# caishiqing/voice-tts

Measured on AMD Instinct MI355X. Metric: audio_seconds_per_second, higher is better.
Workload: dtype bf16

## Files before the change

voice-tts_amd/csrc/gemm_x6.hip:

```cpp
#include "common.h"

namespace ixtts {

typedef float gx_f32x16 __attribute__((ext_vector_type(16)));
typedef __bf16 gx_bf16x8 __attribute__((ext_vector_type(8)));
typedef float gx_f32x4 __attribute__((ext_vector_type(4)));
typedef unsigned int gx_u32x4 __attribute__((ext_vector_type(4)));


__global__ void gemm_x6_pack_kernel(const float* __restrict__ w, uint4* __restrict__ out, int N, int K, int Npad) {
  const long total = (long)(K / 8) * Npad;
  for (long idx = blockIdx.x * (long)blockDim.x + threadIdx.x; idx < total; idx += (long)gridDim.x * blockDim.x) {
    const int n = (int)(idx % Npad);
    const int ko = (int)(idx / Npad);
    float v[8];
#pragma unroll
    for (int e = 0; e < 8; ++e) v[e] = n < N ? w[(long)n * K + ko * 8 + e] : 0.f;
    uint4 ph, pm, pl;
    split8_bf16x3(v, ph, pm, pl);
    const int g = ko >> 1, kh = ko & 1;
    uint4* base = out + ((long)g * 6) * Npad + n;
    base[(long)(0 * 2 + kh) * Npad] = ph;
    base[(long)(1 * 2 + kh) * Npad] = pm;
    base[(long)(2 * 2 + kh) * Npad] = pl;
  }
}

__global__ __launch_bounds__(256) void gemm_x6_split_kernel(const float* __restrict__ a, long lda, uint4* __restrict__ out, int M, int K, long Mpad) {
  __shared__ float tile[64][65];
  const int r0 = blockIdx.x * 64, k0 = blockIdx.y * 64;
  const int t = threadIdx.x;
#pragma unroll
  for (int i = 0; i < 4; ++i) {
    const int r = (t >> 4) + 16 * i, kq = t & 15;
    float4 v = make_float4(0.f, 0.f, 0.f, 0.f);
    if (r0 + r < M) v = *reinterpret_cast<const float4*>(a + (long)(r0 + r) * lda + k0 + 4 * kq);
    tile[r][4 * kq + 0] = v.x; tile[r][4 * kq + 1] = v.y; tile[r][4 * kq + 2] = v.z; tile[r][4 * kq + 3] = v.w;
  }
  __syncthreads();
#pragma unroll
  for (int u = 0; u < 2; ++u) {
    const int r = t & 63, o = (t >> 6) + 4 * u;
    float v[8];
#pragma unroll
    for (int e = 0; e < 8; ++e) v[e] = tile[r][o * 8 + e];
    uint4 ph, pm, pl;
    split8_bf16x3(v, ph, pm, pl);
    const int ko = (k0 >> 3) + o, g = ko >> 1, kh = ko & 1;
    uint4* base = out + ((long)g * 6) * Mpad + r0 + r;
    base[(long)(0 * 2 + kh) * Mpad] = ph;
    base[(long)(1 * 2 + kh) * Mpad] = pm;
    base[(long)(2 * 2 + kh) * Mpad] = pl;
  }
}

struct GemmX6Params {
  const uint4* Ap;
  long Mpad;
  long arow0;
  const uint4* Wp;
  const float* bias;
  float* C;
  long ldc;
  int M, N, Npad, K, accumulate, m_tiles, n_tiles;
  unsigned long long* dbg;
};


template <int MT, int NT, int NST, int DBG = 0>
__global__ __launch_bounds__(256, (NST * (MT + NT) * 6 * 64 * 16 <= 80 * 1024) ? 2 : 1) void gemm_x6_kernel(GemmX6Params p) {
  constexpr int BM = 64 * MT, BN = 64 * NT;
  constexpr int A_UNITS = 6 * BM, W_UNITS = 6 * BN, STAGE = A_UNITS + W_UNITS;
  constexpr int NDMA = (6 * (MT + NT)) / 4;
  static_assert((6 * (MT + NT)) % 4 == 0, "the copies are dealt evenly to the 4 waves");
  constexpr int D = NST - 1;
  extern __shared__ uint4 smem[];

  const int nwg = p.m_tiles * p.n_tiles;
  const int bid = blockIdx.x;
  const int xcd = bid & 7, idx = bid >> 3;
  const int qd = nwg >> 3, rm = nwg & 7;
  const int lin = (xcd < rm ? xcd * (qd + 1) : rm * (qd + 1) + (xcd - rm) * qd) + idx;
  const int m_tile = lin / p.n_tiles, n_tile = lin - m_tile * p.n_tiles;
  const int m0 = m_tile * BM, n0 = n_tile * BN;

  const int tid = threadIdx.x, lane = tid & 63, wave = tid >> 6;
  const int wm = wave >> 1, wn = wave & 1;
  const int l31 = lane & 31, lh = lane >> 5;

  gx_f32x16 acc[MT][NT];
#pragma unroll
  for (int i = 0; i < MT; ++i)
#pragma unroll
    for (int j = 0; j < NT; ++j)
#pragma unroll
      for (int r = 0; r < 16; ++r) acc[i][j][r] = 0.f;

  const uint4* asrc = p.Ap + p.arow0 + m0 + lane;
  const uint4* wsrc = p.Wp + n0 + lane;
  auto issue = [&](int s, uint4* st) {
#pragma unroll
    for (int q = 0; q < NDMA; ++q) {
      const int e = q * 4 + wave;
      if (e < 6 * MT) {
        const int run = e / MT, piece = e % MT;
        __builtin_amdgcn_global_load_lds((const __attribute__((address_space(1))) void*)(asrc + ((long)s * 6 + run) * p.Mpad + piece * 64),
                                         (__attribute__((address_space(3))) void*)(st + run * BM + piece * 64), 16, 0, 0);
      } else {
        const int e2 = e - 6 * MT, run = e2 / NT, piece = e2 % NT;
        __builtin_amdgcn_global_load_lds((const __attribute__((address_space(1))) void*)(wsrc + ((long)s * 6 + run) * p.Npad + piece * 64),
                                         (__attribute__((address_space(3))) void*)(st + A_UNITS + run * BN + piece * 64), 16, 0, 0);
      }
    }
  };

  const int steps = p.K >> 4;
  auto wg_stamp = [&](int k) {
    if constexpr (DBG == 3) {
      if (tid == 0) p.dbg[128 + (long)blockIdx.x * 4 + k] = __builtin_amdgcn_s_memrealtime();
    }
  };
  auto wait_younger = [&](int y) {
    if (y >= 2) asm volatile("s_waitcnt vmcnt(%0)" ::"n"(2 * NDMA) : "memory");
    else if (y == 1) asm volatile("s_waitcnt vmcnt(%0)" ::"n"(NDMA) : "memory");
    else asm volatile("s_waitcnt vmcnt(0)" ::: "memory");
  };
  static_assert(D >= 1 && D <= 3, "1..3 steps of copies in flight behind the one waited for");
  wg_stamp(0);
  for (int t = 0; t < D && t < steps; ++t) issue(t, smem + t * STAGE);
  wait_younger(min(D, steps) - 1);
  __builtin_amdgcn_s_barrier();
  asm volatile("" ::: "memory");
  wg_stamp(1);

  const unsigned base_addr = (unsigned)(uintptr_t)(const __attribute__((address_space(3))) void*)smem;
  int st_cur = 0, st_nxt = D % NST;
  for (int s = 0; s < steps; ++s) {
    auto stamp = [&](int k) {
      if constexpr (DBG == 3) {
        if (blockIdx.x == 0 && tid == 0 && s < 16) {
          p.dbg[s * 8 + k] = __builtin_amdgcn_s_memtime();
          if (k == 0) p.dbg[s * 8 + 7] = __builtin_amdgcn_s_memrealtime();
        }
      }
    };
    stamp(0);
    if (DBG != 1 && s + D < steps) issue(s + D, smem + st_nxt * STAGE);
    stamp(1);
    const unsigned cur_addr = base_addr + (unsigned)(st_cur * STAGE * 16);
    if constexpr (DBG != 2) {
      gx_u32x4 af[3][MT], bf[3][NT];
      const unsigned aaddr = cur_addr + (unsigned)((lh * BM + wm * (32 * MT) + l31) * 16);
      const unsigned waddr = cur_addr + (unsigned)((A_UNITS + lh * BN + wn * (32 * NT) + l31) * 16);
      if constexpr (MT == 4 && NT == 2) {
        asm volatile(
            "ds_read_b128 %0, %18 offset:%20\n ds_read_b128 %1, %18 offset:%21\n ds_read_b128 %2, %18 offset:%22\n ds_read_b128 %3, %18 offset:%23\n"
            "ds_read_b128 %4, %18 offset:%24\n ds_read_b128 %5, %18 offset:%25\n ds_read_b128 %6, %18 offset:%26\n ds_read_b128 %7, %18 offset:%27\n"
            "ds_read_b128 %8, %18 offset:%28\n ds_read_b128 %9, %18 offset:%29\n ds_read_b128 %10, %18 offset:%30\n ds_read_b128 %11, %18 offset:%31\n"
            "ds_read_b128 %12, %19 offset:%32\n ds_read_b128 %13, %19 offset:%33\n ds_read_b128 %14, %19 offset:%34\n ds_read_b128 %15, %19 offset:%35\n"
            "ds_read_b128 %16, %19 offset:%36\n ds_read_b128 %17, %19 offset:%37\n s_waitcnt lgkmcnt(0)"
            : "=&v"(af[0][0]), "=&v"(af[0][1]), "=&v"(af[0][2]), "=&v"(af[0][3]), "=&v"(af[1][0]), "=&v"(af[1][1]), "=&v"(af[1][2]), "=&v"(af[1][3]),
              "=&v"(af[2][0]), "=&v"(af[2][1]), "=&v"(af[2][2]), "=&v"(af[2][3]), "=&v"(bf[0][0]), "=&v"(bf[0][1]), "=&v"(bf[1][0]), "=&v"(bf[1][1]),
              "=&v"(bf[2][0]), "=&v"(bf[2][1])
            : "v"(aaddr), "v"(waddr), "n"((0 * 2 * BM + 0) * 16), "n"((0 * 2 * BM + 32) * 16), "n"((0 * 2 * BM + 64) * 16), "n"((0 * 2 * BM + 96) * 16),
              "n"((1 * 2 * BM + 0) * 16), "n"((1 * 2 * BM + 32) * 16), "n"((1 * 2 * BM + 64) * 16), "n"((1 * 2 * BM + 96) * 16), "n"((2 * 2 * BM + 0) * 16),
              "n"((2 * 2 * BM + 32) * 16), "n"((2 * 2 * BM + 64) * 16), "n"((2 * 2 * BM + 96) * 16), "n"((0 * 2 * BN + 0) * 16), "n"((0 * 2 * BN + 32) * 16),
              "n"((1 * 2 * BN + 0) * 16), "n"((1 * 2 * BN + 32) * 16), "n"((2 * 2 * BN + 0) * 16), "n"((2 * 2 * BN + 32) * 16)
            : "memory");
      } else {
        static_assert(MT == 2 && NT == 2, "fragment block written for 256 x 128 and 128 x 128 tiles");
        asm volatile(
            "ds_read_b128 %0, %12 offset:%14\n ds_read_b128 %1, %12 offset:%15\n ds_read_b128 %2, %12 offset:%16\n ds_read_b128 %3, %12 offset:%17\n"
            "ds_read_b128 %4, %12 offset:%18\n ds_read_b128 %5, %12 offset:%19\n ds_read_b128 %6, %13 offset:%20\n ds_read_b128 %7, %13 offset:%21\n"
            "ds_read_b128 %8, %13 offset:%22\n ds_read_b128 %9, %13 offset:%23\n ds_read_b128 %10, %13 offset:%24\n ds_read_b128 %11, %13 offset:%25\n"
            "s_waitcnt lgkmcnt(0)"
            : "=&v"(af[0][0]), "=&v"(af[0][1]), "=&v"(af[1][0]), "=&v"(af[1][1]), "=&v"(af[2][0]), "=&v"(af[2][1]), "=&v"(bf[0][0]), "=&v"(bf[0][1]),
              "=&v"(bf[1][0]), "=&v"(bf[1][1]), "=&v"(bf[2][0]), "=&v"(bf[2][1])
            : "v"(aaddr), "v"(waddr), "n"((0 * 2 * BM + 0) * 16), "n"((0 * 2 * BM + 32) * 16), "n"((1 * 2 * BM + 0) * 16), "n"((1 * 2 * BM + 32) * 16),
              "n"((2 * 2 * BM + 0) * 16), "n"((2 * 2 * BM + 32) * 16), "n"((0 * 2 * BN + 0) * 16), "n"((0 * 2 * BN + 32) * 16), "n"((1 * 2 * BN + 0) * 16),
              "n"((1 * 2 * BN + 32) * 16), "n"((2 * 2 * BN + 0) * 16), "n"((2 * 2 * BN + 32) * 16)
            : "memory");
      }
      stamp(2);
#pragma unroll
      for (int i = 0; i < MT; ++i)
#pragma unroll
        for (int j = 0; j < NT; ++j) {
          const gx_bf16x8 ah = __builtin_bit_cast(gx_bf16x8, af[0][i]), am = __builtin_bit_cast(gx_bf16x8, af[1][i]), al = __builtin_bit_cast(gx_bf16x8, af[2][i]);
          const gx_bf16x8 bh = __builtin_bit_cast(gx_bf16x8, bf[0][j]), bm = __builtin_bit_cast(gx_bf16x8, bf[1][j]), bl = __builtin_bit_cast(gx_bf16x8, bf[2][j]);
          acc[i][j] = __builtin_amdgcn_mfma_f32_32x32x16_bf16(al, bh, acc[i][j], 0, 0, 0);
          acc[i][j] = __builtin_amdgcn_mfma_f32_32x32x16_bf16(ah, bl, acc[i][j], 0, 0, 0);
          acc[i][j] = __builtin_amdgcn_mfma_f32_32x32x16_bf16(am, bm, acc[i][j], 0, 0, 0);
          acc[i][j] = __builtin_amdgcn_mfma_f32_32x32x16_bf16(am, bh, acc[i][j], 0, 0, 0);
          acc[i][j] = __builtin_amdgcn_mfma_f32_32x32x16_bf16(ah, bm, acc[i][j], 0, 0, 0);
          acc[i][j] = __builtin_amdgcn_mfma_f32_32x32x16_bf16(ah, bh, acc[i][j], 0, 0, 0);
        }
      if constexpr (DBG == 3) asm volatile("" ::"v"(acc[0][0][0]), "v"(acc[MT - 1][NT - 1][15]));
    }
    stamp(3);
    wait_younger(DBG == 1 ? 0 : max(0, min(D - 1, steps - s - 2)));
    stamp(4);
    __builtin_amdgcn_s_barrier();
    asm volatile("" ::: "memory");
    stamp(5);
    st_cur = st_cur + 1 == NST ? 0 : st_cur + 1;
    st_nxt = st_nxt + 1 == NST ? 0 : st_nxt + 1;
  }

  wg_stamp(2);
#pragma unroll
  for (int j = 0; j < NT; ++j) {
    const int col = n0 + wn * (32 * NT) + j * 32 + l31;
    const bool col_ok = col < p.N;
    const float bv = (p.bias != nullptr && col_ok) ? p.bias[col] : 0.f;
#pragma unroll
    for (int i = 0; i < MT; ++i) {
      const int rbase = m0 + wm * (32 * MT) + i * 32 + 4 * lh;
#pragma unroll
      for (int r = 0; r < 16; ++r) {
        const int row = rbase + (r & 3) + 8 * (r >> 2);
        if (col_ok && row < p.M) {
          float* c = p.C + (long)row * p.ldc + col;
          float v = acc[i][j][r] + bv;
          if (p.accumulate) v += *c;
          *c = v;
        }
      }
    }
  }
  if constexpr (DBG == 3) {
    asm volatile("s_waitcnt vmcnt(0)" ::: "memory");
    wg_stamp(3);
  }
}

template <int MT, int NT, int NST, int DBG = 0>
static int launch_gemm_x6(GemmX6Params p, hipStream_t st) {
  constexpr int BM = 64 * MT, BN = 64 * NT;
  constexpr size_t smem = (size_t)NST * (6 * BM + 6 * BN) * 16;
  static_assert(smem <= 160 * 1024, "LDS stages of this tile shape");
  p.m_tiles = ceil_div(p.M, BM);
  p.n_tiles = ceil_div(p.N, BN);
  IX_ARG((long)p.n_tiles * BN <= p.Npad, "gemm_x6: packed weights padded to %d features, the %d-wide tile needs %d", p.Npad, BN, p.n_tiles * BN);
  IX_ARG(p.arow0 + (long)p.m_tiles * BM <= p.Mpad, "gemm_x6: activation planes hold %ld rows, the %d-row tiles reach row %ld", p.Mpad, BM, p.arow0 + (long)p.m_tiles * BM);
  auto kern = gemm_x6_kernel<MT, NT, NST, DBG>;
  static bool done = false;
  if (!done) {
    IX_HIP(hipFuncSetAttribute((const void*)kern, hipFuncAttributeMaxDynamicSharedMemorySize, (int)smem));
    done = true;
  }
  hipLaunchKernelGGL(kern, dim3(p.m_tiles * p.n_tiles), dim3(256), smem, st, p);
  IX_HIP(hipGetLastError());
  return IXTTS_OK;
}

}

using namespace ixtts;

extern "C" size_t ixtts_gemm_x6_packed_bytes(int N, int K) {
  if (N <= 0 || K <= 0 || K % 64) return 0;
  const size_t Npad = (size_t)(N + 255) / 256 * 256;
  return (size_t)(K / 16) * 6 * Npad * 16;
}

extern "C" int ixtts_gemm_x6_pack(const float* w_dev, void* packed_dev, int N, int K, void* stream) {
  IX_ARG(w_dev && packed_dev && N > 0 && K > 0 && K % 64 == 0, "gemm_x6_pack: bad argument (K must be a multiple of 64)");
  const int Npad = (N + 255) / 256 * 256;
  const long total = (long)(K / 8) * Npad;
  hipLaunchKernelGGL(gemm_x6_pack_kernel, dim3((unsigned)std::min<long>((total + 255) / 256, 4096)), dim3(256), 0, (hipStream_t)stream, w_dev,
                     reinterpret_cast<uint4*>(packed_dev), N, K, Npad);
  IX_HIP(hipGetLastError());
  return IXTTS_OK;
}

extern "C" long ixtts_gemm_x6_rows_padded(long rows) { return rows <= 0 ? 0 : (rows + 255) / 256 * 256 + 256; }

extern "C" int ixtts_gemm_x6_split(const float* a_dev, long lda, void* planes_dev, long rows, int K, void* stream) {
  IX_ARG(a_dev && planes_dev && rows > 0 && K > 0 && K % 64 == 0, "gemm_x6_split: bad argument (K must be a multiple of 64)");
  IX_ARG(lda >= K && lda % 4 == 0 && (reinterpret_cast<uintptr_t>(a_dev) & 15) == 0, "gemm_x6_split: rows must be 16-byte aligned (lda %ld)", lda);
  const long Mpad = ixtts_gemm_x6_rows_padded(rows);
  hipLaunchKernelGGL(gemm_x6_split_kernel, dim3((unsigned)(Mpad / 64), K / 64), dim3(256), 0, (hipStream_t)stream, a_dev, lda,
                     reinterpret_cast<uint4*>(planes_dev), (int)rows, K, Mpad);
  IX_HIP(hipGetLastError());
  return IXTTS_OK;
}

extern "C" int ixtts_gemm_x6_f32(const void* a_planes_dev, long rows_total, long row0, const void* packed_dev, const float* bias_dev, float* c_dev,
                                 long ldc, int M, int N, int K, int accumulate, int tile, void* stream) {
  IX_ARG(a_planes_dev && packed_dev && c_dev && M > 0 && N > 0 && K > 0 && K % 64 == 0, "gemm_x6: bad argument (K must be a multiple of 64: the split pass works on 64-wide k blocks)");
  IX_ARG(ldc >= N && row0 >= 0 && row0 + M <= rows_total, "gemm_x6: rows [%ld, %ld) of %ld, ldc %ld", row0, row0 + M, rows_total, ldc);
  GemmX6Params p;
  p.Ap = reinterpret_cast<const uint4*>(a_planes_dev); p.Mpad = ixtts_gemm_x6_rows_padded(rows_total); p.arow0 = row0;
  p.Wp = reinterpret_cast<const uint4*>(packed_dev); p.bias = bias_dev; p.C = c_dev; p.ldc = ldc;
  p.M = M; p.N = N; p.Npad = (N + 255) / 256 * 256; p.K = K; p.accumulate = accumulate ? 1 : 0; p.m_tiles = p.n_tiles = 0;
  p.dbg = (tile == 32 || tile == 33) ? reinterpret_cast<unsigned long long*>(const_cast<float*>(bias_dev)) : nullptr;
  if (p.dbg) p.bias = nullptr;
  hipStream_t st = (hipStream_t)stream;
  if (tile == 0) {
    const long t42 = (long)ceil_div(M, 256) * ceil_div(N, 128);
    tile = t42 >= 140 ? 2 : 3;
  }
  switch (tile) {
    case 2: return launch_gemm_x6<4, 2, 2>(p, st);
    case 3: return launch_gemm_x6<2, 2, 3>(p, st);
    case 4: return launch_gemm_x6<4, 2, 4>(p, st);
    case 5: return launch_gemm_x6<2, 2, 4>(p, st);
    case 12: return launch_gemm_x6<4, 2, 2, 1>(p, st);
    case 22: return launch_gemm_x6<4, 2, 2, 2>(p, st);
    case 32: return launch_gemm_x6<4, 2, 2, 3>(p, st);
    case 33: return launch_gemm_x6<2, 2, 3, 3>(p, st);
  }
  set_error("gemm_x6: tile %d (0 auto; 2 / 3: 256x128 / 128x128, two workgroups per CU; 4 / 5: the same, one per CU with a 4-stage ring)", tile);
  return IXTTS_ERR_ARG;
}
```

voice-tts_amd/s2mel.py:

```python
import math
import os

import torch
import torch.nn.functional as F

from .convs import conv1d

from .weights import fold_weight_norm

S2MEL_CFG = dict(
    hidden_dim=512, num_heads=8, depth=13, in_channels=80, content_dim=512, style_dim=192,
    wavenet_hidden=512, wavenet_layers=8, wavenet_kernel=5, wavenet_dilation_rate=1,
    lr_channels=512, lr_in_channels=1024, lr_n_blocks=4, gpt_dim=1280, codebook_dim=8, codebook_size=8192, semantic_dim=1024,
)


def tiny_s2mel_cfg(**kw):
    c = dict(S2MEL_CFG)
    c.update(hidden_dim=64, num_heads=2, depth=5, content_dim=32, style_dim=12, wavenet_hidden=64, wavenet_layers=3,
             lr_channels=32, lr_in_channels=40, lr_n_blocks=2, gpt_dim=128, codebook_size=8194, semantic_dim=40)
    c.update(kw)
    return c


# ... 90 lines not shown
    ws = torch.empty(nws, device=q.device, dtype=torch.uint8)
    with torch.cuda.device(q.device):
        rc = L.ixtts_attn_full_f32(q.data_ptr(), k.data_ptr(), v.data_ptr(), out.data_ptr(), B, Hh, T, d, q.stride(0), q.stride(1),
                                   q.stride(2), out.stride(0), out.stride(1), out.stride(2), C.c_float(sc), ws.data_ptr(), nws,
                                   _lib.current_stream_ptr())
    _lib.check(rc, "ixtts_attn_full_f32")
    return out


def _lin(x, W, name):
    return F.linear(x, W[name + ".weight"], W.get(name + ".bias"))


def _hip_call(name, *args):
    from . import _lib

    _lib.check(getattr(_lib.lib(), name)(*args, _lib.current_stream_ptr()), name)


def adaln_rmsnorm(x, wb, g, eps=1e-5):
    B, T, H = x.shape
    if x.is_cuda:
        import ctypes as C

        x, wb = x.contiguous(), wb.contiguous()
        out = torch.empty_like(x)
        with torch.cuda.device(x.device):
            _hip_call("ixtts_adaln_rmsnorm_f32", x.data_ptr(), wb.data_ptr(), g.data_ptr(), out.data_ptr(), B, T, H, C.c_float(eps))
        return out
    w, b = wb[:, None, :H], wb[:, None, H:]
    return torch.addcmul(b, w, F.rms_norm(x, (H,), g, eps))


def ln_modulate(x, ss, eps=1e-6):
    B, T, H = x.shape
    if x.is_cuda:
        import ctypes as C

        x, ss = x.contiguous(), ss.contiguous()
        out = torch.empty_like(x)
        with torch.cuda.device(x.device):
            _hip_call("ixtts_ln_modulate_f32", x.data_ptr(), ss.data_ptr(), out.data_ptr(), B, T, H, C.c_float(eps))
        return out
    return F.layer_norm(x, (H,), None, None, eps) * (1 + ss[:, None, H:]) + ss[:, None, :H]


def swiglu(u):
    Fd = u.shape[-1] // 2
    if u.is_cuda:
        u = u.contiguous()
        out = torch.empty(*u.shape[:-1], Fd, device=u.device, dtype=u.dtype)
        with torch.cuda.device(u.device):
            _hip_call("ixtts_swiglu_f32", u.data_ptr(), out.data_ptr(), u.numel() // (2 * Fd), Fd)
        return out
    return F.silu(u[..., :Fd]) * u[..., Fd:]


def wn_gate(a, g, off, C_):
    B, _, T = a.shape
    if a.is_cuda:
        a, g = a.contiguous(), g.contiguous()
        out = torch.empty(B, C_, T, device=a.device, dtype=a.dtype)
        with torch.cuda.device(a.device):
            _hip_call("ixtts_wn_gate_f32", a.data_ptr(), g.data_ptr(), out.data_ptr(), B, C_, T, g.shape[1], off)
        return out
    x = a + g[:, off:off + 2 * C_, None]
    return torch.tanh(x[:, :C_]) * torch.sigmoid(x[:, C_:])


def wn_gate_rows(a, g, off, C_, rows_per_batch):
    rows, B = a.shape[0], g.shape[0]
    if a.is_cuda:
        a, g = a.contiguous(), g.contiguous()
        out = torch.empty(rows, C_, device=a.device, dtype=a.dtype)
        with torch.cuda.device(a.device):
            _hip_call("ixtts_wn_gate_rows_f32", a.data_ptr(), g.data_ptr(), out.data_ptr(), rows, C_, rows_per_batch, B, g.shape[1], off)
        return out
    b = (torch.arange(rows, device=a.device) // rows_per_batch).clamp(max=B - 1)
    x = a + g[b, off:off + 2 * C_]
    return torch.tanh(x[:, :C_]) * torch.sigmoid(x[:, C_:])


def reflect_halo_rows(p, T, left, right):
    B, _, C_ = p.shape
    if p.is_cuda:
        assert p.is_contiguous()
        with torch.cuda.device(p.device):
            _hip_call("ixtts_reflect_halo_rows_f32", p.data_ptr(), B, T, C_, left, right)
        return p
    if left:
        p[:, :left] = p[:, left + 1:2 * left + 1].flip(1)
    if right:
        p[:, left + T:] = p[:, left + T - 1 - right:left + T - 1].flip(1)
    return p


TUNED_GEMMS = os.path.join(os.path.dirname(os.path.abspath(__file__)), "tunable", "gfx950_s2mel.csv")


def use_tuned_gemms(path=TUNED_GEMMS):
    if not torch.cuda.is_available():
        return False
    import torch.cuda.tunable as tn

    tn.enable(True)
    tn.tuning_enable(os.environ.get("IXTTS_TUNE") == "1")
    try:
        import tempfile

        tn.set_filename(os.path.join(tempfile.gettempdir(), "ixtts_tunableop_online.csv"))
    except Exception:
        pass
    try:
        return bool(os.path.isfile(path) and tn.read_file(path))
    except Exception:
        return False


_TUNED_T0, _TUNED_TH0 = 2322, 1909
_tuned_lengths = set()


def extend_tuned_gemms(T, Th, path=TUNED_GEMMS):
    if (T, Th) in _tuned_lengths or (T, Th) == (_TUNED_T0, _TUNED_TH0):
        return False
    _tuned_lengths.add((T, Th))
    import tempfile

    import torch.cuda.tunable as tn

    sub = {str(2 * _TUNED_T0): str(2 * T), str(_TUNED_T0): str(T), str(_TUNED_TH0): str(Th), str(2 * _TUNED_TH0): str(2 * Th),
           str(2 * _TUNED_TH0 + 4): str(2 * Th + 4)}
    head, rows = [], []
    for line in open(path).read().splitlines():
        f = line.split(",")
        if f[0] == "Validator":
            head.append(line)
        elif len(f) >= 4 and f[2] != "Default" and f[0].endswith("_TN"):
            toks = f[1].split("_")
            if any(t in sub for t in toks):
                rows.append(",".join([f[0], "_".join(sub.get(t, t) for t in toks)] + f[2:]))
    if not rows:
        return False
    with tempfile.NamedTemporaryFile("w", suffix=".csv", delete=False) as fh:
        fh.write("\n".join(head + rows) + "\n")
    try:
        return bool(tn.read_file(fh.name))
    except Exception:
        return False
    finally:
        os.unlink(fh.name)


class S2Mel:
    def __init__(self, W, cfg=S2MEL_CFG, device="cpu"):
        self.cfg = dict(cfg)
        self.device = torch.device(device)
        self.tuned_gemms = False
        if self.device.type == "cuda" and os.environ.get("IXTTS_NO_TUNED_GEMMS") != "1":
            self.tuned_gemms = use_tuned_gemms()
        W = fold_weight_norm(dict(W))
        self.W = {k: v.to(self.device, torch.float32) for k, v in W.items()}
        H = cfg["hidden_dim"]
        self.head_dim = H // cfg["num_heads"]
        half = 128
        self.t_freqs = torch.exp(-math.log(10000.0) * torch.arange(half, dtype=torch.float32) / half).to(self.device)
        self._rope = None
        W, C_, L = self.W, cfg["in_channels"], cfg["depth"]
        t = "cfm.estimator.transformer."
        self.w13 = [torch.cat([W[t + f"layers.{i}.feed_forward.w1.weight"], W[t + f"layers.{i}.feed_forward.w3.weight"]], 0).contiguous() for i in range(L)]
        self.skip_w = {i: (W[t + f"layers.{i}.skip_in_linear.weight"][:, :H].contiguous(), W[t + f"layers.{i}.skip_in_linear.weight"][:, H:].contiguous())
                       for i in range(L // 2 + 1, L)}
        names = [t + f"layers.{i}.{n}" for i in range(L) for n in ("attention_norm", "ffn_norm")] + [t + "norm"]
        self.proj_w = torch.cat([W[n + ".project_layer.weight"] for n in names], 0).contiguous()
        self.proj_b = torch.cat([W[n + ".project_layer.bias"] for n in names], 0).contiguous()
        mw = W["cfm.estimator.cond_x_merge_linear.weight"]
        self.merge_x, self.merge_rest = mw[:, :C_].contiguous(), mw[:, C_:].contiguous()
        wn = "cfm.estimator.wavenet."
        self.wn_taps = [[W[wn + f"in_layers.{i}.conv.conv.weight"][:, :, j].contiguous() for j in range(cfg["wavenet_kernel"])]
                        for i in range(cfg["wavenet_layers"])]
        nl, Hw = cfg["wavenet_layers"], cfg["wavenet_hidden"]
        self.wn_r1, self.wn_r2, self.wn_bin = [], [], []
        carry = torch.zeros(Hw, device=self.device)
        self.wn_out_bias = torch.zeros(Hw, device=self.device)
        for i in range(nl):
            rw, rb = W[wn + f"res_skip_layers.{i}.conv.conv.weight"][:, :, 0], W[wn + f"res_skip_layers.{i}.conv.conv.bias"]
            self.wn_bin.append(W[wn + f"in_layers.{i}.conv.conv.bias"] + sum(self.wn_taps[i]) @ carry)
            if i < nl - 1:
                self.wn_r1.append(rw[:Hw].contiguous())
                self.wn_r2.append(rw[Hw:].contiguous())
                carry = carry + rb[:Hw]
                self.wn_out_bias = self.wn_out_bias + rb[Hw:]
            else:
                self.wn_r1.append(None)
                self.wn_r2.append(rw.contiguous())
                self.wn_out_bias = self.wn_out_bias + rb
        sw = W["cfm.estimator.skip_linear.weight"]
        self.skipl_res, self.skipl_x = sw[:, :H].contiguous(), sw[:, H:].contiguous()

    def gpt_layer(self, latent):
        x = _lin(latent, self.W, "gpt_layer.0")
        x = _lin(x, self.W, "gpt_layer.1")
        return _lin(x, self.W, "gpt_layer.2")

    def vq2emb(self, codes):
        emb = self.W["quantizer.codebook.weight"][codes.long()]
        out = conv1d(emb.transpose(1, 2), self.W["quantizer.out_project.weight"], self.W["quantizer.out_project.bias"])
        return out.transpose(1, 2)

    def length_regulator(self, x, ylens):
        W = self.W
        x = _lin(x, W, "length_regulator.content_in_proj")
        T = int(ylens.max())
        x = F.interpolate(x.transpose(1, 2).contiguous(), size=T, mode="nearest")
        for i in range(self.cfg["lr_n_blocks"]):
            x = conv1d(x, W[f"length_regulator.model.{3 * i}.weight"], W[f"length_regulator.model.{3 * i}.bias"], padding=1)
            x = F.group_norm(x, 1, W[f"length_regulator.model.{3 * i + 1}.weight"], W[f"length_regulator.model.{3 * i + 1}.bias"], 1e-5)
            x = F.mish(x)
        n = 3 * self.cfg["lr_n_blocks"]
        x = conv1d(x, W[f"length_regulator.model.{n}.weight"], W[f"length_regulator.model.{n}.bias"])
        mask = (torch.arange(T, device=x.device).unsqueeze(0) < ylens.unsqueeze(1)).unsqueeze(-1)
        return x.transpose(1, 2) * mask

    def _t_embed(self, t, prefix):
        args = 1000.0 * t[:, None].float() * self.t_freqs[None]
        emb = torch.cat([torch.cos(args), torch.sin(args)], dim=-1)
        h = F.silu(_lin(emb, self.W, prefix + ".mlp.0"))
        return _lin(h, self.W, prefix + ".mlp.2")

    def _rope_cache(self, T):
        if self._rope is None or self._rope.shape[0] < T:
            n = self.head_dim
            freqs = 1.0 / (10000.0 ** (torch.arange(0, n, 2)[: n // 2].float() / n))
            ang = torch.outer(torch.arange(max(T, 64)).float(), freqs)
            self._rope = torch.polar(torch.ones_like(ang), ang).to(self.device)
        return self._rope[:T]

    @staticmethod
    def _rotary(x, fc):
        xc = torch.view_as_complex(x.reshape(*x.shape[:-1], -1, 2))
        return torch.view_as_real(xc * fc.view(1, fc.shape[0], 1, fc.shape[1])).flatten(3)

    def _attention(self, qkv, B, T, mask):
        H, nh, hd = self.cfg["hidden_dim"], self.cfg["num_heads"], self.head_dim
        fc = self._rope_cache(T)
        if mask is None and hd == 64 and qkv.is_cuda:
            with torch.cuda.device(qkv.device):
                _hip_call("ixtts_rope_qk_f32", qkv.data_ptr(), torch.view_as_real(fc).data_ptr(), B, T, H, hd)
            v4 = qkv.view(B, T, 3, nh, hd)
            return attn_full(v4[:, :, 0], v4[:, :, 1], v4[:, :, 2]).reshape(B * T, H)
        q, k, v = qkv.view(B, T, 3 * H).split([H, H, H], dim=-1)
        q = self._rotary(q.reshape(B, T, nh, hd), fc)
        k = self._rotary(k.reshape(B, T, nh, hd), fc)
        v = v.reshape(B, T, nh, hd)
        y = F.scaled_dot_product_attention(q.transpose(1, 2), k.transpose(1, 2), v.transpose(1, 2), attn_mask=mask, dropout_p=0.0)
        return y.transpose(1, 2).reshape(B * T, H)

    def _transformer(self, x, c, mask):
        W, cfg = self.W, self.cfg
        B, T, H = x.shape
        L = cfg["depth"]
        wb_all = F.linear(c, self.proj_w, self.proj_b).view(B, 2 * L + 1, 2 * H).transpose(0, 1).contiguous()
        x = x.reshape(B * T, H)
        skips = []
        for i in range(L):
            p = f"cfm.estimator.transformer.layers.{i}."
            if i > L // 2:
                wa, wb_ = self.skip_w[i]
                x = F.linear(skips.pop(), wb_, W[p + "skip_in_linear.bias"]).addmm_(x, wa.t())
            a = adaln_rmsnorm(x.view(B, T, H), wb_all[2 * i], W[p + "attention_norm.norm.weight"])
            y = self._attention(F.linear(a.view(B * T, H), W[p + "attention.wqkv.weight"]), B, T, mask)
            h = torch.addmm(x, y, W[p + "attention.wo.weight"].t()) if 0 < i <= L // 2 else x.addmm_(y, W[p + "attention.wo.weight"].t())
            f = adaln_rmsnorm(h.view(B, T, H), wb_all[2 * i + 1], W[p + "ffn_norm.norm.weight"])
            x = h.addmm_(swiglu(F.linear(f.view(B * T, H), self.w13[i])), W[p + "feed_forward.w2.weight"].t())
            if i < L // 2:
                skips.append(x)
        return adaln_rmsnorm(x.view(B, T, H), wb_all[2 * L], W["cfm.estimator.transformer.norm.norm.weight"])

    def _wavenet(self, x, x_mask, g, full):
        W, cfg = self.W, self.cfg
        Hw, nl, k = cfg["wavenet_hidden"], cfg["wavenet_layers"], cfg["wavenet_kernel"]
        p = "cfm.estimator.wavenet."
        g = F.linear(g, W[p + "cond_layer.conv.conv.weight"][:, :, 0], W[p + "cond_layer.conv.conv.bias"])
        out = None
        for i in range(nl):
            d = cfg["wavenet_dilation_rate"] ** i
            tot = (k - 1) * d
            right = tot // 2
            xin = _pad_reflect(x, tot - right, right)
            if x.is_cuda:
                wk, T_ = self.wn_taps[i], x.shape[-1]
                acc = W[p + f"in_layers.{i}.conv.conv.bias"][None, :, None].expand(x.shape[0], -1, T_)
                for j in range(k):
                    wj, xj = wk[j].expand(x.shape[0], -1, -1), xin[:, :, j * d:j * d + T_]
                    acc = torch.baddbmm(acc, wj, xj) if j == 0 else acc.baddbmm_(wj, xj)
                xin = acc
            else:
                xin = conv1d(xin, W[p + f"in_layers.{i}.conv.conv.weight"], W[p + f"in_layers.{i}.conv.conv.bias"], dilation=d)
            acts = wn_gate(xin, g, i * 2 * Hw, Hw)
            rs = conv1d(acts, W[p + f"res_skip_layers.{i}.conv.conv.weight"], W[p + f"res_skip_layers.{i}.conv.conv.bias"])
            if i < nl - 1:
                x = x + rs[:, :Hw]
                if not full:
                    x = x * x_mask
                out = rs[:, Hw:] if out is None else out + rs[:, Hw:]
            else:
                out = rs if out is None else out + rs
        return out if full else out * x_mask

    def _wavenet_gemm(self, x, g):
        W, cfg = self.W, self.cfg
        Hw, nl, k = cfg["wavenet_hidden"], cfg["wavenet_layers"], cfg["wavenet_kernel"]
        B, _, T_ = x.shape
        p = "cfm.estimator.wavenet."
        g = F.linear(g, W[p + "cond_layer.conv.conv.weight"][:, :, 0], W[p + "cond_layer.conv.conv.bias"])
        x = x.contiguous()
        out = None
        for i in range(nl):
            d = cfg["wavenet_dilation_rate"] ** i
            tot = (k - 1) * d
            right = tot // 2
            xin = _pad_reflect(x, tot - right, right)
            acc = self.wn_bin[i][None, :, None].expand(B, -1, T_)
            for j in range(k):
                wj, xj = self.wn_taps[i][j].expand(B, -1, -1), xin[:, :, j * d:j * d + T_]
                acc = torch.baddbmm(acc, wj, xj) if j == 0 else acc.baddbmm_(wj, xj)
            acts = wn_gate(acc, g, i * 2 * Hw, Hw)
            if i < nl - 1:
                x = x.baddbmm_(self.wn_r1[i].expand(B, -1, -1), acts)
            r2 = self.wn_r2[i].expand(B, -1, -1)
            out = torch.bmm(r2, acts) if out is None else out.baddbmm_(r2, acts)
        return out

    def _wavenet_rows(self, h, g):
        W, cfg = self.W, self.cfg
        Hw, nl, k = cfg["wavenet_hidden"], cfg["wavenet_layers"], cfg["wavenet_kernel"]
        assert cfg["wavenet_dilation_rate"] == 1
        B, T_, _ = h.shape
        p = "cfm.estimator.wavenet."
        g = F.linear(g, W[p + "cond_layer.conv.conv.weight"][:, :, 0], W[p + "cond_layer.conv.conv.bias"])
        tot = k - 1
        right = tot // 2
        left = tot - right
        Tp = T_ + tot
        P = torch.empty(B, Tp, Hw, device=h.device, dtype=h.dtype)
        P[:, left:left + T_] = h
        P2 = P.view(B * Tp, Hw)
        M = B * Tp - tot
        centre = P2[left:left + M]
        out = torch.empty(B * Tp, Hw, device=h.device, dtype=h.dtype)
        for i in range(nl):
            reflect_halo_rows(P, T_, left, right)
            acc = torch.addmm(self.wn_bin[i], P2[:M], self.wn_taps[i][0].t())
            for j in range(1, k):
                acc.addmm_(P2[j:j + M], self.wn_taps[i][j].t())
            acts = wn_gate_rows(acc, g, i * 2 * Hw, Hw, Tp)
            if i < nl - 1:
                centre.addmm_(acts, self.wn_r1[i].t())
            if i == 0:
                torch.mm(acts, self.wn_r2[i].t(), out=out[:M])
            else:
                out[:M].addmm_(acts, self.wn_r2[i].t())
        return out.view(B, Tp, Hw)[:, :T_]

    def dit_prepare(self, prompt_x, x_lens, style, cond):
        W = self.W
        e = "cfm.estimator."
        B, _, T = prompt_x.shape
        cond = _lin(cond, W, e + "cond_projection")
        rest = torch.cat([prompt_x.transpose(1, 2), cond, style[:, None, :].expand(B, T, style.shape[-1])], dim=-1)
        base = F.linear(rest, self.merge_rest, W[e + "cond_x_merge_linear.bias"])
        x_mask = (torch.arange(T, device=prompt_x.device).unsqueeze(0) < x_lens.unsqueeze(1)).unsqueeze(1)
        full = int(x_lens.min()) >= T
        if full:
            attn_mask = None
        else:
            attn_mask = x_mask[:, None, :].expand(x_mask.shape[0], 1, T, T)
            if attn_mask.shape[0] != B:
                attn_mask = attn_mask.expand(B, 1, T, T)
        return dict(B=B, T=T, base=base, x_mask=x_mask.to(base.dtype), attn_mask=attn_mask, full=full)

    def dit_step(self, ctx, x, t, out_from=0):
        W, cfg = self.W, self.cfg
        e = "cfm.estimator."
        B, T, base = ctx["B"], ctx["T"], ctx["base"]
        xt = x.transpose(1, 2)
        t1 = self._t_embed(t, e + "t_embedder")
        x_in = base + F.linear(xt, self.merge_x)
        x_res = self._transformer(x_in, t1, ctx["attn_mask"])
        halo = sum((cfg["wavenet_kernel"] - 1) * cfg["wavenet_dilation_rate"] ** i for i in range(cfg["wavenet_layers"])) // 2 + 1
        lo = max(0, out_from - halo) if (ctx["full"] and out_from > 0) else 0
        if lo > 0:
            x_res, xt = x_res[:, lo:], xt[:, lo:]
        Th = T - lo
        if self.tuned_gemms and os.environ.get("IXTTS_TUNED_ANY_LENGTH", "1") == "1":
            extend_tuned_gemms(T, Th)
        x_res = F.linear(x_res, self.skipl_res, W[e + "skip_linear.bias"]) + F.linear(xt, self.skipl_x)
        h = _lin(x_res, W, e + "conv1")
        t2 = self._t_embed(t, e + "t_embedder2")
        gemm_form = h.is_cuda and ctx["full"] and Th > 2 * cfg["wavenet_kernel"] * cfg["wavenet_dilation_rate"] ** (cfg["wavenet_layers"] - 1)
        if gemm_form and cfg["wavenet_dilation_rate"] == 1:
            h = self._wavenet_rows(h, t2) + F.linear(x_res, W[e + "res_projection.weight"], W[e + "res_projection.bias"] + self.wn_out_bias)
        elif gemm_form:
            h = self._wavenet_gemm(h.transpose(1, 2), t2).transpose(1, 2) + F.linear(x_res, W[e + "res_projection.weight"],
                                                                                     W[e + "res_projection.bias"] + self.wn_out_bias)
        else:
            mask = ctx["x_mask"][:, :, lo:] if lo > 0 else ctx["x_mask"]
            h = self._wavenet(h.transpose(1, 2), mask, t2, ctx["full"]).transpose(1, 2) + _lin(x_res, W, e + "res_projection")
        ss = _lin(F.silu(t1), W, e + "final_layer.adaLN_modulation.1")
        h = ln_modulate(h, ss)
        h = _lin(h, W, e + "final_layer.linear").transpose(1, 2)
        out = conv1d(h, W[e + "conv2.weight"], W[e + "conv2.bias"])
        return out[:, :, out_from - lo:] if out_from > 0 else out

    def dit(self, x, prompt_x, x_lens, t, style, cond):
        return self.dit_step(self.dit_prepare(prompt_x, x_lens, style, cond), x, t)

    @torch.no_grad()
    def cfm_inference(self, mu, x_lens, prompt, style, n_timesteps=25, inference_cfg_rate=0.7, noise=None, temperature=1.0):
        B, T = mu.shape[0], mu.shape[1]
        assert B == 1, "CFM inference is batch-1 (as the reference)"
        z = (torch.randn(B, self.cfg["in_channels"], T, device=mu.device) if noise is None else noise.to(mu.device, torch.float32)) * temperature
        t_span = torch.linspace(0, 1, n_timesteps + 1, device=mu.device)
        x = z.clone()
        Tp = prompt.shape[-1]
        prompt_x = torch.zeros_like(x)
        prompt_x[..., :Tp] = prompt[..., :Tp]
# ... 34 lines not shown
```

Measured before the change: 39.78.

## Route S2Mel wqkv and w13 projections through split-bf16 x6 GEMM with 8-wave tiles

Generalizes the x6 GEMM kernel to configurable wave grids (WM x WN) and adds 8-wave 256x256 and 256x128 tile variants. S2Mel now pre-packs the wqkv and fused w1/w3 weights into the three-way bf16 split format. It sends those projections through the x6 kernel, choosing the tile by row count, instead of the fp32 library linear. The aim is to replace fp32 GEMMs with MFMA-based emulated-fp32 matmuls, at the cost of extra packing memory and activation packing per call.

Result: faster. 40.19 (median of 6 runs) (+1.0%).

```diff
diff --git a/voice-tts_amd/csrc/gemm_x6.hip b/voice-tts_amd/csrc/gemm_x6.hip
--- a/voice-tts_amd/csrc/gemm_x6.hip
+++ b/voice-tts_amd/csrc/gemm_x6.hip
@@ -67,12 +67,15 @@
 };
 
 
-template <int MT, int NT, int NST, int DBG = 0>
-__global__ __launch_bounds__(256, (NST * (MT + NT) * 6 * 64 * 16 <= 80 * 1024) ? 2 : 1) void gemm_x6_kernel(GemmX6Params p) {
-  constexpr int BM = 64 * MT, BN = 64 * NT;
+template <int MT, int NT, int NST, int DBG = 0, int WM = 2, int WN = 2>
+__global__ __launch_bounds__(64 * WM * WN, WM * WN > 4 ? 1 : (NST * (MT + NT) * 6 * 64 * 16 <= 80 * 1024) ? 2 : 1) void gemm_x6_kernel(GemmX6Params p) {
+  constexpr int NW = WM * WN;
+  constexpr int BM = 32 * MT * WM, BN = 32 * NT * WN;
   constexpr int A_UNITS = 6 * BM, W_UNITS = 6 * BN, STAGE = A_UNITS + W_UNITS;
-  constexpr int NDMA = (6 * (MT + NT)) / 4;
-  static_assert((6 * (MT + NT)) % 4 == 0, "the copies are dealt evenly to the 4 waves");
+  constexpr int PA = BM / 64, PW = BN / 64;
+  constexpr int NPIECE = 6 * (PA + PW);
+  constexpr int NDMA = (NPIECE + NW - 1) / NW;
+  static_assert(BM % 64 == 0 && BN % 64 == 0, "tiles of whole 64-unit pieces");
   constexpr int D = NST - 1;
   extern __shared__ uint4 smem[];
 
@@ -85,7 +88,7 @@
   const int m0 = m_tile * BM, n0 = n_tile * BN;
 
   const int tid = threadIdx.x, lane = tid & 63, wave = tid >> 6;
-  const int wm = wave >> 1, wn = wave & 1;
+  const int wm = wave / WN, wn = wave % WN;
   const int l31 = lane & 31, lh = lane >> 5;
 
   gx_f32x16 acc[MT][NT];
@@ -101,13 +104,13 @@
   auto issue = [&](int s, uint4* st) {
 #pragma unroll
     for (int q = 0; q < NDMA; ++q) {
-      const int e = q * 4 + wave;
-      if (e < 6 * MT) {
-        const int run = e / MT, piece = e % MT;
+      const int e = min(q * NW + wave, NPIECE - 1);
+      if (e < 6 * PA) {
+        const int run = e / PA, piece = e % PA;
         __builtin_amdgcn_global_load_lds((const __attribute__((address_space(1))) void*)(asrc + ((long)s * 6 + run) * p.Mpad + piece * 64),
                                          (__attribute__((address_space(3))) void*)(st + run * BM + piece * 64), 16, 0, 0);
       } else {
-        const int e2 = e - 6 * MT, run = e2 / NT, piece = e2 % NT;
+        const int e2 = e - 6 * PA, run = e2 / PW, piece = e2 % PW;
         __builtin_amdgcn_global_load_lds((const __attribute__((address_space(1))) void*)(wsrc + ((long)s * 6 + run) * p.Npad + piece * 64),
                                          (__attribute__((address_space(3))) void*)(st + A_UNITS + run * BN + piece * 64), 16, 0, 0);
       }
@@ -133,6 +136,54 @@
   asm volatile("" ::: "memory");
   wg_stamp(1);
 
+  auto read_frags = [&](unsigned cur_addr, gx_u32x4 (&af)[3][MT], gx_u32x4 (&bf)[3][NT]) {
+    const unsigned aaddr = cur_addr + (unsigned)((lh * BM + wm * (32 * MT) + l31) * 16);
+    const unsigned waddr = cur_addr + (unsigned)((A_UNITS + lh * BN + wn * (32 * NT) + l31) * 16);
+    if constexpr (MT == 4 && NT == 2) {
+      asm volatile(
+          "ds_read_b128 %0, %18 offset:%20\n ds_read_b128 %1, %18 offset:%21\n ds_read_b128 %2, %18 offset:%22\n ds_read_b128 %3, %18 offset:%23\n"
+          "ds_read_b128 %4, %18 offset:%24\n ds_read_b128 %5, %18 offset:%25\n ds_read_b128 %6, %18 offset:%26\n ds_read_b128 %7, %18 offset:%27\n"
+          "ds_read_b128 %8, %18 offset:%28\n ds_read_b128 %9, %18 offset:%29\n ds_read_b128 %10, %18 offset:%30\n ds_read_b128 %11, %18 offset:%31\n"
+          "ds_read_b128 %12, %19 offset:%32\n ds_read_b128 %13, %19 offset:%33\n ds_read_b128 %14, %19 offset:%34\n ds_read_b128 %15, %19 offset:%35\n"
+          "ds_read_b128 %16, %19 offset:%36\n ds_read_b128 %17, %19 offset:%37\n s_waitcnt lgkmcnt(0)"
+          : "=&v"(af[0][0]), "=&v"(af[0][1]), "=&v"(af[0][2]), "=&v"(af[0][3]), "=&v"(af[1][0]), "=&v"(af[1][1]), "=&v"(af[1][2]), "=&v"(af[1][3]),
+            "=&v"(af[2][0]), "=&v"(af[2][1]), "=&v"(af[2][2]), "=&v"(af[2][3]), "=&v"(bf[0][0]), "=&v"(bf[0][1]), "=&v"(bf[1][0]), "=&v"(bf[1][1]),
+            "=&v"(bf[2][0]), "=&v"(bf[2][1])
+          : "v"(aaddr), "v"(waddr), "n"((0 * 2 * BM + 0) * 16), "n"((0 * 2 * BM + 32) * 16), "n"((0 * 2 * BM + 64) * 16), "n"((0 * 2 * BM + 96) * 16),
+            "n"((1 * 2 * BM + 0) * 16), "n"((1 * 2 * BM + 32) * 16), "n"((1 * 2 * BM + 64) * 16), "n"((1 * 2 * BM + 96) * 16), "n"((2 * 2 * BM + 0) * 16),
+            "n"((2 * 2 * BM + 32) * 16), "n"((2 * 2 * BM + 64) * 16), "n"((2 * 2 * BM + 96) * 16), "n"((0 * 2 * BN + 0) * 16), "n"((0 * 2 * BN + 32) * 16),
+            "n"((1 * 2 * BN + 0) * 16), "n"((1 * 2 * BN + 32) * 16), "n"((2 * 2 * BN + 0) * 16), "n"((2 * 2 * BN + 32) * 16)
+          : "memory");
+    } else {
+      static_assert(MT == 2 && NT == 2, "fragment block written for 256 x 128 and 128 x 128 tiles");
+      asm volatile(
+          "ds_read_b128 %0, %12 offset:%14\n ds_read_b128 %1, %12 offset:%15\n ds_read_b128 %2, %12 offset:%16\n ds_read_b128 %3, %12 offset:%17\n"
+          "ds_read_b128 %4, %12 offset:%18\n ds_read_b128 %5, %12 offset:%19\n ds_read_b128 %6, %13 offset:%20\n ds_read_b128 %7, %13 offset:%21\n"
+          "ds_read_b128 %8, %13 offset:%22\n ds_read_b128 %9, %13 offset:%23\n ds_read_b128 %10, %13 offset:%24\n ds_read_b128 %11, %13 offset:%25\n"
+          "s_waitcnt lgkmcnt(0)"
+          : "=&v"(af[0][0]), "=&v"(af[0][1]), "=&v"(af[1][0]), "=&v"(af[1][1]), "=&v"(af[2][0]), "=&v"(af[2][1]), "=&v"(bf[0][0]), "=&v"(bf[0][1]),
+            "=&v"(bf[1][0]), "=&v"(bf[1][1]), "=&v"(bf[2][0]), "=&v"(bf[2][1])
+          : "v"(aaddr), "v"(waddr), "n"((0 * 2 * BM + 0) * 16), "n"((0 * 2 * BM + 32) * 16), "n"((1 * 2 * BM + 0) * 16), "n"((1 * 2 * BM + 32) * 16),
+            "n"((2 * 2 * BM + 0) * 16), "n"((2 * 2 * BM + 32) * 16), "n"((0 * 2 * BN + 0) * 16), "n"((0 * 2 * BN + 32) * 16), "n"((1 * 2 * BN + 0) * 16),
+            "n"((1 * 2 * BN + 32) * 16), "n"((2 * 2 * BN + 0) * 16), "n"((2 * 2 * BN + 32) * 16)
+          : "memory");
+    }
+  };
+  auto mfmas = [&](const gx_u32x4 (&af)[3][MT], const gx_u32x4 (&bf)[3][NT]) {
+#pragma unroll
+    for (int i = 0; i < MT; ++i)
+#pragma unroll
+      for (int j = 0; j < NT; ++j) {
+        const gx_bf16x8 ah = __builtin_bit_cast(gx_bf16x8, af[0][i]), am = __builtin_bit_cast(gx_bf16x8, af[1][i]), al = __builtin_bit_cast(gx_bf16x8, af[2][i]);
+        const gx_bf16x8 bh = __builtin_bit_cast(gx_bf16x8, bf[0][j]), bm = __builtin_bit_cast(gx_bf16x8, bf[1][j]), bl = __builtin_bit_cast(gx_bf16x8, bf[2][j]);
+        acc[i][j] = __builtin_amdgcn_mfma_f32_32x32x16_bf16(al, bh, acc[i][j], 0, 0, 0);
+        acc[i][j] = __builtin_amdgcn_mfma_f32_32x32x16_bf16(ah, bl, acc[i][j], 0, 0, 0);
+        acc[i][j] = __builtin_amdgcn_mfma_f32_32x32x16_bf16(am, bm, acc[i][j], 0, 0, 0);
+        acc[i][j] = __builtin_amdgcn_mfma_f32_32x32x16_bf16(am, bh, acc[i][j], 0, 0, 0);
+        acc[i][j] = __builtin_amdgcn_mfma_f32_32x32x16_bf16(ah, bm, acc[i][j], 0, 0, 0);
+        acc[i][j] = __builtin_amdgcn_mfma_f32_32x32x16_bf16(ah, bh, acc[i][j], 0, 0, 0);
+      }
+  };
   const unsigned base_addr = (unsigned)(uintptr_t)(const __attribute__((address_space(3))) void*)smem;
   int st_cur = 0, st_nxt = D % NST;
   for (int s = 0; s < steps; ++s) {
@@ -150,51 +201,9 @@
     const unsigned cur_addr = base_addr + (unsigned)(st_cur * STAGE * 16);
     if constexpr (DBG != 2) {
       gx_u32x4 af[3][MT], bf[3][NT];
-      const unsigned aaddr = cur_addr + (unsigned)((lh * BM + wm * (32 * MT) + l31) * 16);
-      const unsigned waddr = cur_addr + (unsigned)((A_UNITS + lh * BN + wn * (32 * NT) + l31) * 16);
-      if constexpr (MT == 4 && NT == 2) {
-        asm volatile(
-            "ds_read_b128 %0, %18 offset:%20\n ds_read_b128 %1, %18 offset:%21\n ds_read_b128 %2, %18 offset:%22\n ds_read_b128 %3, %18 offset:%23\n"
-            "ds_read_b128 %4, %18 offset:%24\n ds_read_b128 %5, %18 offset:%25\n ds_read_b128 %6, %18 offset:%26\n ds_read_b128 %7, %18 offset:%27\n"
-            "ds_read_b128 %8, %18 offset:%28\n ds_read_b128 %9, %18 offset:%29\n ds_read_b128 %10, %18 offset:%30\n ds_read_b128 %11, %18 offset:%31\n"
-            "ds_read_b128 %12, %19 offset:%32\n ds_read_b128 %13, %19 offset:%33\n ds_read_b128 %14, %19 offset:%34\n ds_read_b128 %15, %19 offset:%35\n"
-            "ds_read_b128 %16, %19 offset:%36\n ds_read_b128 %17, %19 offset:%37\n s_waitcnt lgkmcnt(0)"
-            : "=&v"(af[0][0]), "=&v"(af[0][1]), "=&v"(af[0][2]), "=&v"(af[0][3]), "=&v"(af[1][0]), "=&v"(af[1][1]), "=&v"(af[1][2]), "=&v"(af[1][3]),
-              "=&v"(af[2][0]), "=&v"(af[2][1]), "=&v"(af[2][2]), "=&v"(af[2][3]), "=&v"(bf[0][0]), "=&v"(bf[0][1]), "=&v"(bf[1][0]), "=&v"(bf[1][1]),
-              "=&v"(bf[2][0]), "=&v"(bf[2][1])
-            : "v"(aaddr), "v"(waddr), "n"((0 * 2 * BM + 0) * 16), "n"((0 * 2 * BM + 32) * 16), "n"((0 * 2 * BM + 64) * 16), "n"((0 * 2 * BM + 96) * 16),
-              "n"((1 * 2 * BM + 0) * 16), "n"((1 * 2 * BM + 32) * 16), "n"((1 * 2 * BM + 64) * 16), "n"((1 * 2 * BM + 96) * 16), "n"((2 * 2 * BM + 0) * 16),
-              "n"((2 * 2 * BM + 32) * 16), "n"((2 * 2 * BM + 64) * 16), "n"((2 * 2 * BM + 96) * 16), "n"((0 * 2 * BN + 0) * 16), "n"((0 * 2 * BN + 32) * 16),
-              "n"((1 * 2 * BN + 0) * 16), "n"((1 * 2 * BN + 32) * 16), "n"((2 * 2 * BN + 0) * 16), "n"((2 * 2 * BN + 32) * 16)
-            : "memory");
-      } else {
-        static_assert(MT == 2 && NT == 2, "fragment block written for 256 x 128 and 128 x 128 tiles");
-        asm volatile(
-            "ds_read_b128 %0, %12 offset:%14\n ds_read_b128 %1, %12 offset:%15\n ds_read_b128 %2, %12 offset:%16\n ds_read_b128 %3, %12 offset:%17\n"
-            "ds_read_b128 %4, %12 offset:%18\n ds_read_b128 %5, %12 offset:%19\n ds_read_b128 %6, %13 offset:%20\n ds_read_b128 %7, %13 offset:%21\n"
-            "ds_read_b128 %8, %13 offset:%22\n ds_read_b128 %9, %13 offset:%23\n ds_read_b128 %10, %13 offset:%24\n ds_read_b128 %11, %13 offset:%25\n"
-            "s_waitcnt lgkmcnt(0)"
-            : "=&v"(af[0][0]), "=&v"(af[0][1]), "=&v"(af[1][0]), "=&v"(af[1][1]), "=&v"(af[2][0]), "=&v"(af[2][1]), "=&v"(bf[0][0]), "=&v"(bf[0][1]),
-              "=&v"(bf[1][0]), "=&v"(bf[1][1]), "=&v"(bf[2][0]), "=&v"(bf[2][1])
-            : "v"(aaddr), "v"(waddr), "n"((0 * 2 * BM + 0) * 16), "n"((0 * 2 * BM + 32) * 16), "n"((1 * 2 * BM + 0) * 16), "n"((1 * 2 * BM + 32) * 16),
-              "n"((2 * 2 * BM + 0) * 16), "n"((2 * 2 * BM + 32) * 16), "n"((0 * 2 * BN + 0) * 16), "n"((0 * 2 * BN + 32) * 16), "n"((1 * 2 * BN + 0) * 16),
-              "n"((1 * 2 * BN + 32) * 16), "n"((2 * 2 * BN + 0) * 16), "n"((2 * 2 * BN + 32) * 16)
-            : "memory");
-      }
+      read_frags(cur_addr, af, bf);
       stamp(2);
-#pragma unroll
-      for (int i = 0; i < MT; ++i)
-#pragma unroll
-        for (int j = 0; j < NT; ++j) {
-          const gx_bf16x8 ah = __builtin_bit_cast(gx_bf16x8, af[0][i]), am = __builtin_bit_cast(gx_bf16x8, af[1][i]), al = __builtin_bit_cast(gx_bf16x8, af[2][i]);
-          const gx_bf16x8 bh = __builtin_bit_cast(gx_bf16x8, bf[0][j]), bm = __builtin_bit_cast(gx_bf16x8, bf[1][j]), bl = __builtin_bit_cast(gx_bf16x8, bf[2][j]);
-          acc[i][j] = __builtin_amdgcn_mfma_f32_32x32x16_bf16(al, bh, acc[i][j], 0, 0, 0);
-          acc[i][j] = __builtin_amdgcn_mfma_f32_32x32x16_bf16(ah, bl, acc[i][j], 0, 0, 0);
-          acc[i][j] = __builtin_amdgcn_mfma_f32_32x32x16_bf16(am, bm, acc[i][j], 0, 0, 0);
-          acc[i][j] = __builtin_amdgcn_mfma_f32_32x32x16_bf16(am, bh, acc[i][j], 0, 0, 0);
-          acc[i][j] = __builtin_amdgcn_mfma_f32_32x32x16_bf16(ah, bm, acc[i][j], 0, 0, 0);
-          acc[i][j] = __builtin_amdgcn_mfma_f32_32x32x16_bf16(ah, bh, acc[i][j], 0, 0, 0);
-        }
+      mfmas(af, bf);
       if constexpr (DBG == 3) asm volatile("" ::"v"(acc[0][0][0]), "v"(acc[MT - 1][NT - 1][15]));
     }
     stamp(3);
@@ -234,22 +243,22 @@
   }
 }
 
-template <int MT, int NT, int NST, int DBG = 0>
+template <int MT, int NT, int NST, int DBG = 0, int WM = 2, int WN = 2>
 static int launch_gemm_x6(GemmX6Params p, hipStream_t st) {
-  constexpr int BM = 64 * MT, BN = 64 * NT;
+  constexpr int BM = 32 * MT * WM, BN = 32 * NT * WN;
   constexpr size_t smem = (size_t)NST * (6 * BM + 6 * BN) * 16;
   static_assert(smem <= 160 * 1024, "LDS stages of this tile shape");
   p.m_tiles = ceil_div(p.M, BM);
   p.n_tiles = ceil_div(p.N, BN);
   IX_ARG((long)p.n_tiles * BN <= p.Npad, "gemm_x6: packed weights padded to %d features, the %d-wide tile needs %d", p.Npad, BN, p.n_tiles * BN);
   IX_ARG(p.arow0 + (long)p.m_tiles * BM <= p.Mpad, "gemm_x6: activation planes hold %ld rows, the %d-row tiles reach row %ld", p.Mpad, BM, p.arow0 + (long)p.m_tiles * BM);
-  auto kern = gemm_x6_kernel<MT, NT, NST, DBG>;
+  auto kern = gemm_x6_kernel<MT, NT, NST, DBG, WM, WN>;
   static bool done = false;
   if (!done) {
     IX_HIP(hipFuncSetAttribute((const void*)kern, hipFuncAttributeMaxDynamicSharedMemorySize, (int)smem));
     done = true;
   }
-  hipLaunchKernelGGL(kern, dim3(p.m_tiles * p.n_tiles), dim3(256), smem, st, p);
+  hipLaunchKernelGGL(kern, dim3(p.m_tiles * p.n_tiles), dim3(64 * WM * WN), smem, st, p);
   IX_HIP(hipGetLastError());
   return IXTTS_OK;
 }
@@ -306,11 +315,14 @@
     case 3: return launch_gemm_x6<2, 2, 3>(p, st);
     case 4: return launch_gemm_x6<4, 2, 4>(p, st);
     case 5: return launch_gemm_x6<2, 2, 4>(p, st);
+    case 6: return launch_gemm_x6<4, 2, 3, 0, 2, 4>(p, st);
+    case 7: return launch_gemm_x6<2, 2, 3, 0, 4, 2>(p, st);
     case 12: return launch_gemm_x6<4, 2, 2, 1>(p, st);
     case 22: return launch_gemm_x6<4, 2, 2, 2>(p, st);
     case 32: return launch_gemm_x6<4, 2, 2, 3>(p, st);
     case 33: return launch_gemm_x6<2, 2, 3, 3>(p, st);
   }
-  set_error("gemm_x6: tile %d (0 auto; 2 / 3: 256x128 / 128x128, two workgroups per CU; 4 / 5: the same, one per CU with a 4-stage ring)", tile);
+  set_error("gemm_x6: tile %d (0 auto; 2 / 3: 256x128 / 128x128, two workgroups per CU; 4 / 5: the same, one per CU with a 4-stage ring; "
+            "6 / 7: 256x256 / 256x128, 8 waves)", tile);
   return IXTTS_ERR_ARG;
 }
diff --git a/voice-tts_amd/s2mel.py b/voice-tts_amd/s2mel.py
--- a/voice-tts_amd/s2mel.py
+++ b/voice-tts_amd/s2mel.py
@@ -266,6 +266,9 @@
         os.unlink(fh.name)
 
 
+X6_ROUTES = {"w13": ((4096, 6), (0, 7)), "wqkv": ((4096, 7), (0, 3))}
+
+
 class S2Mel:
     def __init__(self, W, cfg=S2MEL_CFG, device="cpu"):
         self.cfg = dict(cfg)
@@ -283,6 +286,15 @@
         W, C_, L = self.W, cfg["in_channels"], cfg["depth"]
         t = "cfm.estimator.transformer."
         self.w13 = [torch.cat([W[t + f"layers.{i}.feed_forward.w1.weight"], W[t + f"layers.{i}.feed_forward.w3.weight"]], 0).contiguous() for i in range(L)]
+        self.x6 = {}
+        if self.device.type == "cuda" and os.environ.get("IXTTS_S2MEL_GEMM", "x6") != "library":
+            from . import gemm as G
+
+            for i in range(L):
+                if "w13" in X6_ROUTES:
+                    self.x6[("w13", i)] = G.PackedLinear(self.w13[i])
+                if "wqkv" in X6_ROUTES:
+                    self.x6[("wqkv", i)] = G.PackedLinear(W[t + f"layers.{i}.attention.wqkv.weight"])
         self.skip_w = {i: (W[t + f"layers.{i}.skip_in_linear.weight"][:, :H].contiguous(), W[t + f"layers.{i}.skip_in_linear.weight"][:, H:].contiguous())
                        for i in range(L // 2 + 1, L)}
         names = [t + f"layers.{i}.{n}" for i in range(L) for n in ("attention_norm", "ffn_norm")] + [t + "norm"]
@@ -370,6 +382,15 @@
         y = F.scaled_dot_product_attention(q.transpose(1, 2), k.transpose(1, 2), v.transpose(1, 2), attn_mask=mask, dropout_p=0.0)
         return y.transpose(1, 2).reshape(B * T, H)
 
+    def _linear(self, x, route, i, weight):
+        pl = self.x6.get((route, i))
+        if pl is None:
+            return F.linear(x, weight)
+        from . import gemm as G
+
+        M = x.shape[0]
+        return G.linear(x, pl, tile=next(t for m0, t in X6_ROUTES[route] if M >= m0))
+
     def _transformer(self, x, c, mask):
         W, cfg = self.W, self.cfg
         B, T, H = x.shape
@@ -383,10 +404,10 @@
                 wa, wb_ = self.skip_w[i]
                 x = F.linear(skips.pop(), wb_, W[p + "skip_in_linear.bias"]).addmm_(x, wa.t())
             a = adaln_rmsnorm(x.view(B, T, H), wb_all[2 * i], W[p + "attention_norm.norm.weight"])
-            y = self._attention(F.linear(a.view(B * T, H), W[p + "attention.wqkv.weight"]), B, T, mask)
+            y = self._attention(self._linear(a.view(B * T, H), "wqkv", i, W[p + "attention.wqkv.weight"]), B, T, mask)
             h = torch.addmm(x, y, W[p + "attention.wo.weight"].t()) if 0 < i <= L // 2 else x.addmm_(y, W[p + "attention.wo.weight"].t())
             f = adaln_rmsnorm(h.view(B, T, H), wb_all[2 * i + 1], W[p + "ffn_norm.norm.weight"])
-            x = h.addmm_(swiglu(F.linear(f.view(B * T, H), self.w13[i])), W[p + "feed_forward.w2.weight"].t())
+            x = h.addmm_(swiglu(self._linear(f.view(B * T, H), "w13", i, self.w13[i])), W[p + "feed_forward.w2.weight"].t())
             if i < L // 2:
                 skips.append(x)
         return adaln_rmsnorm(x.view(B, T, H), wb_all[2 * L], W["cfm.estimator.transformer.norm.norm.weight"])
```
